# se-hwan/landing-controller

Measured on AMD Instinct MI355X. Metric: landing NLPs solved/sec (SRBM, N=40, batch), higher is better.
Workload: dtype f64

## Files before the change

### landing-controller_amd/csrc/solver_capi.inc

```

namespace {

struct StageTab {
  std::vector<int> tg_ab, tg_start, tg_term, gm_start, gm_term, a_term, r_start, r_term;
  int nu;
  std::vector<std::array<int, 4>> cterm;
  std::vector<std::array<int, 4>> rterm;
  std::vector<unsigned long long> cloc;
  bool operator==(const StageTab& o) const {
    return nu == o.nu && tg_ab == o.tg_ab && tg_start == o.tg_start && tg_term == o.tg_term && gm_start == o.gm_start &&
           gm_term == o.gm_term && a_term == o.a_term && r_start == o.r_start && r_term == o.r_term && cloc == o.cloc;
  }
};

int w_index(const Layout& L, int k, long long c) {
  const int N = L.N;
  if (c >= L.x_X(k) && c < L.x_X(k) + 12) return (int)(c - L.x_X(k));
  if (c >= L.x_U(k) && c < L.x_U(k) + 24) { const int j = (int)(c - L.x_U(k)); return j < 12 ? 12 + j : 24 + (j - 12); }
  if (k < N - 1 && c >= L.x_U(k + 1) && c < L.x_U(k + 1) + 12) return 36 + (int)(c - L.x_U(k + 1));
  return -1;
}
int jpos(const Layout& L, int k, long long c, long long idx) {
  if (c >= L.x_X(k) && c < L.x_X(k) + 12) return landing::NZ_JX + (int)(idx - L.jx(k));
  if (c >= L.x_U(k) && c < L.x_U(k) + 24) return landing::NZ_JU + (int)(idx - L.ju(k));
// ... 89 lines not shown
      };
      for (int i = 0; i < 12; ++i) add_c(i, i, i);
      for (int l = 0; l < 4; ++l) for (int a = 0; a < 3; ++a) add_c(a, 12 + 3 * l + a, 12 + 3 * l + a);
      for (int j = 0; j < 12; ++j) add_c(12 + j, 12 + j, 24 + j);
      for (int j = 0; j < 12; ++j) add_c(24 + j, 24 + j, 36 + j);
    }
    T.tg_start.push_back(0);
    for (auto& kv : tg) {
      T.tg_ab.push_back(kv.first.first | (kv.first.second << 8));
      for (auto& t : kv.second) { T.tg_term.push_back(t[0]); T.tg_term.push_back(t[1]); T.tg_term.push_back(t[2]); }
      T.tg_start.push_back((int)T.tg_term.size() / 3);
    }
    T.gm_start.push_back(0);
    for (int a = 0; a < 48; ++a) {
      for (auto& t : gm[a]) { T.gm_term.push_back(t[0]); T.gm_term.push_back(t[1]); }
      T.gm_start.push_back((int)T.gm_term.size() / 2);
    }
    {
      const int base = k * landing::COND_STRIDE;
      if ((int)T.tg_ab.size() > landing::COND_GAM || (int)T.a_term.size() / 3 > landing::COND_STRIDE - landing::COND_AH) return -7;
      int slot = 0;
      for (auto& kv : tg) {
        for (size_t i = 0; i < kv.second.size(); ++i) {
          const auto& t = kv.second[i];
          const int dst = (i + 1 == kv.second.size()) ? base + slot : -1;
          if (t[0] < 0) T.cterm.push_back({-1, pos2idx.at(t[1]), -1, dst});
          else T.cterm.push_back({g0 + t[0], pos2idx.at(t[1]), pos2idx.at(t[2]), dst});
        }
        ++slot;
      }
      for (int a = 0; a < 48; ++a) {
        if (gm[a].empty()) { T.cterm.push_back({-3, 0, -1, base + landing::COND_GAM + a}); continue; }
        for (size_t i = 0; i < gm[a].size(); ++i)
          T.cterm.push_back({g0 + gm[a][i][0], pos2idx.at(gm[a][i][1]), -1, (i + 1 == gm[a].size()) ? base + landing::COND_GAM + a : -1});
      }
      for (size_t i = 0; i < T.a_term.size() / 3; ++i) T.cterm.push_back({-2, pos2idx.at(T.a_term[3 * i]), -1, base + landing::COND_AH + (int)i});
    }
    for (auto& t : T.cterm) {
      int sa = 0, oa = 0, sb = 0, ob = 0;
      const bool has_b = t[2] >= 0;
      if (t[0] != -3 && !encode_jh(L, k, t[1], sa, oa)) return -9;
      if (has_b && !encode_jh(L, k, t[2], sb, ob)) return -9;
      const int rtype = t[0] >= 0 ? 0 : (t[0] == -1 ? 1 : (t[0] == -2 ? 2 : 3));
      const int rowq = t[0] >= 0 ? t[0] - g0 : 0;
      if (rowq < 0 || rowq >= 128) return -9;
      const int dstl = t[3] >= 0 ? t[3] - k * landing::COND_STRIDE : 0;
      if (dstl < 0 || dstl >= 1024) return -9;
      T.cloc.push_back(landing::cterm_pack(sa, oa, sb, ob, has_b, rowq, rtype, dstl, t[3] >= 0));
    }
    for (int ab : T.tg_ab) pat_g[k].insert(ab);
    for (size_t i = 0; i < T.a_term.size() / 3; ++i) pat_a[k].insert(T.a_term[3 * i + 1] * 64 + T.a_term[3 * i + 2]);
    for (auto& t : T.rterm) { rterms.push_back(t[0]); rterms.push_back(t[1]); rterms.push_back(t[2]); rterms.push_back(t[3]); }
    T.cterm.clear(); T.rterm.clear();
    int id = -1;
    for (size_t u = 0; u < uniq.size(); ++u) if (uniq[u] == T) { id = (int)u; break; }
    if (id < 0) { id = (int)uniq.size(); uniq.push_back(T); }
    which[k] = id;
  }
  int zero_each = 0;
  for (int k = N - 2; k >= 0; --k)
    if (!std::includes(pat_g[k].begin(), pat_g[k].end(), pat_g[k + 1].begin(), pat_g[k + 1].end()) ||
        !std::includes(pat_a[k].begin(), pat_a[k].end(), pat_a[k + 1].begin(), pat_a[k + 1].end())) zero_each = 1;
  if (zero_each) return -8;
  data.clear();
  std::vector<int> off(uniq.size());
  for (size_t u = 0; u < uniq.size(); ++u) {
    const StageTab& T = uniq[u];
    off[u] = (int)data.size();
    const int h = (int)data.size();
    data.resize(data.size() + 16, 0);
    auto put = [&](const std::vector<int>& v) { const int o = (int)data.size(); data.insert(data.end(), v.begin(), v.end()); return o; };
    data[h + 0] = (int)T.tg_ab.size();
    data[h + 1] = put(T.tg_ab); data[h + 2] = put(T.tg_start); data[h + 3] = put(T.tg_term);
    data[h + 4] = put(T.gm_start); data[h + 5] = put(T.gm_term);
    data[h + 6] = (int)T.a_term.size() / 3; data[h + 7] = put(T.a_term);
    data[h + 8] = put(T.r_start); data[h + 9] = put(T.r_term);
    data[h + 10] = T.nu;
    data[h + 11] = zero_each;
  }
  for (int k = 0; k < N; ++k) stage_tab[k] = off[which[k]];
  {
    using landing::Lds;
    const int NTH = landing::SOLVER_THREADS;
    const int oG = (int)offsetof(Lds, G), oGam = (int)offsetof(Lds, gam), oAh = (int)offsetof(Lds, Ah), oCx = (int)offsetof(Lds, jhl), oCarry = (int)offsetof(Lds, carry), oDump = (int)offsetof(Lds, dump);
    auto cx = [&](int pos) { return oCx + 8 * pos; };
    int ch = 0;
    for (size_t u = 0; u < uniq.size(); ++u) ch = std::max(ch, ((int)uniq[u].cloc.size() + NTH - 1) / NTH);
    struct Piece { std::vector<std::array<int, 3>> ops; int d; bool ah; };
    std::vector<std::vector<std::vector<unsigned long long>>> lists(uniq.size(), std::vector<std::vector<unsigned long long>>(NTH));
    ccomb.assign(uniq.size() * (size_t)NTH, 0ull);
    c_ml = 0;
    for (size_t u = 0; u < uniq.size(); ++u) {
      const StageTab& T = uniq[u];
      const auto& v = T.cloc; const int n = (int)v.size();
      if (n == 0 || !landing::cterm_closes(v[n - 1])) return -11;
      std::vector<Piece> pieces, cur;
      int nslot = 0, ncomb = 0;
      Piece pc_; pc_.d = 0; pc_.ah = false;
      for (int i = 0; i < n; ++i) {
        const unsigned lo = (unsigned)v[i], hi = (unsigned)(v[i] >> 32);
        const int pa = (int)(lo & 2047u), pb0 = (int)((lo >> 11) & 2047u), rowq = (int)((lo >> 23) & 127u), rtype = (int)(lo >> 30), dst = (int)(hi & 1023u);
        const bool has_b = (lo >> 22) & 1u, closes = landing::cterm_closes(v[i]);
        const int pb = has_b ? pb0 : landing::CX_ONE;
        const int pc = rtype == 0 ? landing::CX_SR + rowq + (has_b ? 0 : 104) : (rtype == 1 ? landing::CX_ONE : (rtype == 2 ? landing::CX_MONE : landing::CX_ZERO));
        if (i % ch == 0 && !pc_.ops.empty()) { cur.push_back(pc_); pc_.ops.clear(); }
        pc_.ops.push_back({cx(pa), cx(pb), cx(pc)});
        if (!closes) continue;
        int d; bool ah = false;
        if (dst < landing::COND_GAM) {
          if (dst >= (int)T.tg_ab.size()) return -12;
          const int a0 = T.tg_ab[dst] & 255, b0 = T.tg_ab[dst] >> 8;
          if (a0 >= 48 || b0 >= 48) return -12;
          d = oG + 8 * (std::min(a0, b0) * landing::GS + std::max(a0, b0));
        } else if (dst < landing::COND_AH) d = oGam + 8 * (dst - landing::COND_GAM);
        else {
          const int q = dst - landing::COND_AH;
          if (3 * q + 2 >= (int)T.a_term.size()) return -12;
          d = oAh + 8 * (T.a_term[3 * q + 1] * landing::YS + T.a_term[3 * q + 2]); ah = true;
        }
        cur.push_back(pc_); pc_.ops.clear();
        if (cur.size() == 1) { cur[0].d = d; cur[0].ah = ah; pieces.push_back(cur[0]); }
        else {
          if (cur.size() > 7 || nslot + (int)cur.size() > landing::ASM_NSLOT || ncomb >= NTH) return -13;
          ccomb[u * NTH + ncomb++] = landing::acomb_pack((int)cur.size(), oCarry + 8 * nslot, d, ah);
          for (auto& q : cur) { q.d = oCarry + 8 * nslot; q.ah = false; ++nslot; pieces.push_back(q); }
        }
        cur.clear();
      }
      std::vector<int> order(pieces.size());
      for (size_t i = 0; i < order.size(); ++i) order[i] = (int)i;
      std::stable_sort(order.begin(), order.end(), [&](int x, int y) { return pieces[x].ops.size() > pieces[y].ops.size(); });
      std::vector<int> load(NTH, 0);
      for (int di : order) {
        const int l = (int)(std::min_element(load.begin(), load.end()) - load.begin());
        const Piece& q = pieces[di];
        for (size_t i = 0; i < q.ops.size(); ++i) {
          const bool lastt = i + 1 == q.ops.size();
          lists[u][l].push_back(landing::aterm_pack(q.ops[i][0], q.ops[i][1], q.ops[i][2], lastt ? q.d : oDump + 8 * (l & 63), !lastt, lastt && q.ah));
        }
        load[l] += (int)q.ops.size();
      }
      c_ml = std::max(c_ml, *std::max_element(load.begin(), load.end()));
    }
    c_ml = (c_ml + landing::ATAB_TB - 1) / landing::ATAB_TB * landing::ATAB_TB;
    if (c_ml > landing::ATAB_LTMAX) return -10;
    ctab.assign(uniq.size() * (size_t)c_ml * NTH, 0ull);
    for (size_t u = 0; u < uniq.size(); ++u)
      for (int l = 0; l < NTH; ++l)
        for (int j = 0; j < c_ml; ++j)
          ctab[(u * c_ml + j) * NTH + l] = j < (int)lists[u][l].size() ? lists[u][l][j]
                                           : landing::aterm_pack(cx(landing::CX_ZERO), cx(landing::CX_ONE), cx(landing::CX_ONE), oDump + 8 * (l & 63), true, false);
    ctype.assign(N, 0);
    std::vector<int> cnt(uniq.size(), 0);
    for (int k = 0; k < N; ++k) { ctype[k] = which[k]; cnt[which[k]]++; }
    c_mid = (int)(std::max_element(cnt.begin(), cnt.end()) - cnt.begin());
  }
  auto chunk_at = [](const std::vector<int>& terms, int dstcol, std::vector<int>& start) {
    const int n = (int)terms.size() / 4, NTH = landing::SOLVER_THREADS;
    start.assign(NTH + 1, n);
    start[0] = 0;
    for (int t = 1; t < NTH; ++t) {
      int want = (int)((long long)n * t / NTH);
      if (want < start[t - 1]) want = start[t - 1];
      while (want < n && want > 0 && terms[4 * (want - 1) + dstcol] < 0) ++want;
      start[t] = want;
    }
  };
  chunk_at(rterms, 2, rstart);
  auto interleave = [](std::vector<int>& terms, std::vector<int>& start, const std::array<int, 4>& pad) {
    const int NTH = landing::SOLVER_THREADS;
    int maxlen = 0;
    for (int t = 0; t < NTH; ++t) maxlen = std::max(maxlen, start[t + 1] - start[t]);
    std::vector<int> out((size_t)maxlen * NTH * 4);
    for (int j = 0; j < maxlen; ++j) for (int t = 0; t < NTH; ++t) {
      const int e = start[t] + j;
      for (int q = 0; q < 4; ++q) out[((size_t)j * NTH + t) * 4 + q] = (e < start[t + 1]) ? terms[4 * (size_t)e + q] : pad[q];
    }
    terms.swap(out);
    start.assign(1, maxlen);
  };
  for (size_t i = 0; i < rterms.size() / 4; ++i) rterms[4 * i + 3] = 1;
  interleave(rterms, rstart, {0, 0, -1, 0});
  {
    const size_t n = rterms.size() / 4;
    std::vector<int> packed(2 * n);
    for (size_t i = 0; i < n; ++i) {
      const int ij = rterms[4 * i], ix = rterms[4 * i + 1], ir = rterms[4 * i + 2], valid = rterms[4 * i + 3];
      if (ij < 0 || ij > 0xffff || ix < 0 || ix > 0xffff || ir > 0xffff) return -18;
      const unsigned long long rec = (unsigned long long)ij | ((unsigned long long)ix << 16) | ((unsigned long long)(ir >= 0 ? ir : 0) << 32) |
                                     ((unsigned long long)(ir >= 0 ? 1 : 0) << 48) | ((unsigned long long)(valid ? 1 : 0) << 49);
      memcpy(&packed[2 * i], &rec, 8);
    }
    rterms.swap(packed);
  }
  return 0;
}

// ... 614 lines not shown
```

### landing-controller_amd/csrc/solver_kernels.hip

```cpp
#include <hip/hip_runtime.h>
#include <math.h>
#include <type_traits>

#include "../../include/landing_nlp.h"
#include "ipm_core.hpp"


namespace landing {

constexpr int NZ_JX = 0, NZ_JU = 157, NZ_JUN = 385, NZ_HX = 613, NZ_HU = 642, NZ_HUN = 802, NZ_TOT = 962;
constexpr int GS = 49;
constexpr int PS = 25;
constexpr int YS = 37;
constexpr int RIC_K = 0, RIC_KAP = 576, RIC_MT = 600, RIC_MV = 888, RIC_PX = 900, RIC_PV = 1188, RIC_STRIDE = 1200;
constexpr int RIC_FWD0 = 288, RIC_FWDN = 612;
constexpr int FILT_CAP = 64;
constexpr int SOLVER_NMAX = 96;
constexpr int ES = 26;
constexpr int SOLVER_THREADS = 256;
constexpr int COND_GAM = 480, COND_AH = 528, COND_STRIDE = 704;
constexpr int RCG = 36;
constexpr int RUNC = 48;

constexpr int CTAB_MLMAX = 6;
// ... 10 lines not shown
constexpr int ASM_NSLOT = 512;

constexpr int EXIT_REC = 8;
inline size_t member_stride(const Layout& L) {
  return (size_t)4 * L.nx + (size_t)20 * L.ng + L.nnz_jac + L.nnz_hess + (size_t)L.N * RUNC + (size_t)(L.N + 1) * RIC_STRIDE + (size_t)L.N * RCG + EXIT_REC;
}

enum { PH_EVAL = 0, PH_ERR, PH_SIGRHO, PH_BACK, PH_FWD, PH_DUAL, PH_LS, PH_ACCEPT, PH_NFACT, PH_NTRIAL, PH_NITER, PH_NSTAGE_OK, PH_B_ASM, PH_NSTAGE, PH_B_ELIM, PH_B_POST,
       PH_COUNT = 16 };
#define PROF_ADD(slot, tstart) do { if (SH.prof_on) { const long long n_ = (long long)wall_clock64(); if (threadIdx.x == 0) { SH.prof[slot] += (double)(n_ - (tstart)); (tstart) = n_; } } } while (0)

enum { EMU_ACC_FAST = 0, EMU_ACC_FAST_CLIP, EMU_ACC_FIRST_REJECTED, EMU_ACC_BACKTRACK, EMU_ACC_CORR, EMU_ACC_FALLBACK, EMU_ACC_FEAS, EMU_ACC_N };
#ifndef __HIPCC__
constexpr int EMU_ACC_MAXB = 64;
static int emu_acc[EMU_ACC_MAXB][EMU_ACC_N];
#define LANDING_EMU_COUNT(m, what) do { if ((m) < EMU_ACC_MAXB) emu_acc[m][what]++; } while (0)
static int emu_fused_on = 1;
#define LANDING_EMU_FUSED_ON (emu_fused_on != 0)
extern "C" void landing_emu_set_fused(int on) { emu_fused_on = on; }
extern "C" int landing_emu_accept_counts(int m, int* counts) {
  if (m < 0 || m >= EMU_ACC_MAXB || !counts) return -1;
  for (int i = 0; i < EMU_ACC_N; ++i) counts[i] = emu_acc[m][i];
  return 0;
}
#else
#define LANDING_EMU_COUNT(m, what) ((void)0)
#define LANDING_EMU_FUSED_ON true
#endif

struct SolveArgs {
  Layout L; int B; landing_solver_opts o; double* prof;
  const double* p; const double* x0;
  double* x_out; double* f_out; double* lam_out; int* status; int* iters; double* kkt;
  double* ws; size_t ws_stride;
  const unsigned long long* rterm; int rlen;
  const unsigned long long* ctab; const int* ctype; int c_ml, c_mid;
  const unsigned long long* ccomb;
  const int* edge_map;
  const int* order;
};

struct MemberMem {
  double *x, *xt, *dx, *gx;
  double *g, *gt, *s, *ds, *zL, *zU, *y, *yn, *sig, *rho;
  double *J, *H, *Hc, *ric, *cond;
  double *en, *ep, *wn, *wp;
  double *sig2, *rho2, *s2, *zL2, *zU2, *y2;
};
constexpr int MEMBER_MEM_PTRS = 29;
static_assert(sizeof(MemberMem) == MEMBER_MEM_PTRS * sizeof(double*) && std::is_standard_layout<MemberMem>::value && std::is_trivially_copyable<MemberMem>::value,
              "live_mem() walks MemberMem as an array of double*: nothing but double* members");

__device__ __forceinline__ MemberMem carve(const Layout& L, double* w) {
  MemberMem M;
  M.x = w; w += L.nx; M.xt = w; w += L.nx; M.dx = w; w += L.nx; M.gx = w; w += L.nx;
  M.g = w; w += L.ng; M.gt = w; w += L.ng; M.s = w; w += L.ng; M.ds = w; w += L.ng;
  M.zL = w; w += L.ng; M.zU = w; w += L.ng;
  M.y = w; w += L.ng; M.yn = w; w += L.ng;
  M.sig = w; w += L.ng; M.rho = w; w += L.ng;
  M.J = w; w += L.nnz_jac; M.H = w; w += L.nnz_hess; M.Hc = w; w += (size_t)L.N * RUNC; M.ric = w; w += (size_t)(L.N + 1) * RIC_STRIDE; M.cond = w; w += (size_t)L.N * RCG;
  M.en = w; w += L.ng; M.ep = w; w += L.ng; M.wn = w; w += L.ng; M.wp = w; w += L.ng;
  M.sig2 = w; w += L.ng; M.rho2 = w; w += L.ng;
  M.s2 = w; w += L.ng; M.zL2 = w; w += L.ng; M.zU2 = w; w += L.ng; M.y2 = w;
  return M;
}

__host__ __device__ __forceinline__ void mem_accept_swap(MemberMem& M) {
  double* t;
#define LANDING_SWAP(a, b) t = M.a; M.a = M.b; M.b = t
  LANDING_SWAP(s, s2); LANDING_SWAP(zL, zL2); LANDING_SWAP(zU, zU2); LANDING_SWAP(y, y2); LANDING_SWAP(sig, sig2); LANDING_SWAP(rho, rho2);
  LANDING_SWAP(g, gt); LANDING_SWAP(x, xt);
#undef LANDING_SWAP
}


constexpr int FWD_DXL_NMAX = 64;
constexpr int XCH = 112 * 4;
static_assert(2 * XCH >= 24 * YS, "A1 also holds Y (24 x YS)");
struct Lds {
  double G[48 * GS];
  double P[24 * PS];
  double A1[2 * XCH];
  double Ah[2 * 12 * YS];
  double gam[48], pv[24], q[24], bv[2 * 12], sig[24], w[48], dinv[24];
  double red[(SOLVER_THREADS / 64) * 9];
  double filt_th[FILT_CAP], filt_ph[FILT_CAP];
  double prof[32];
  int flag;
  int segb[SOLVER_NMAX * 8];
  double carry[ASM_NSLOT];
  double rcl[RCG];
  double jhl[CX_LEN];
  double dump[64];
  const unsigned long long* ctab; const unsigned long long* ccomb; int c_ml, c_mid, rc_on;
  double bnd_lb[36 + 2 * 104], bnd_ub[36 + 2 * 104];
  MemberMem M; Layout L; const double* p; int prof_on;
  IpmCtl ks;
  int clip_now, jamrun, action, fact_failed;
  int first_trial, fast;
  double nxt[6];
  unsigned long long atab_mid[ATAB_LTMAX * SOLVER_THREADS];
  unsigned long long acomb_mid[SOLVER_THREADS];
};
__shared__ Lds SH;
__device__ __forceinline__ MemberMem live_mem() {
  MemberMem M = SH.M;
#if defined(__HIP_DEVICE_COMPILE__)
  double** q = reinterpret_cast<double**>(&M);
#pragma unroll
  for (int i = 0; i < MEMBER_MEM_PTRS; ++i) {
    const unsigned long long a = (unsigned long long)q[i];
    const unsigned lo = (unsigned)__builtin_amdgcn_readfirstlane((int)(unsigned)a), hi = (unsigned)__builtin_amdgcn_readfirstlane((int)(unsigned)(a >> 32));
    q[i] = (double*)((unsigned long long)lo | ((unsigned long long)hi << 32));
  }
#endif
  return M;
}
static_assert(36 * FWD_DXL_NMAX + 12 <= 24 * PS + 2 * XCH + 2 * 12 * YS && offsetof(Lds, A1) == offsetof(Lds, P) + sizeof(double) * 24 * PS && offsetof(Lds, Ah) == offsetof(Lds, A1) + sizeof(double) * 2 * XCH,
              "dx (x layout, N <= FWD_DXL_NMAX) fits the adjacent arrays [P | A1 | A^] (forward_pass / row_products)");
static_assert(offsetof(Lds, atab_mid) <= 65528, "the assembly tables address G, A^, gamma, cx, the partial sums and the dump slots with 16-bit byte offsets");
__host__ __device__ inline unsigned long long aterm_pack(int pa, int pb, int pc, int d, bool keep, bool ah) {
  const unsigned lo = (unsigned)pa | ((unsigned)pb << 16);
  const unsigned hi = (unsigned)pc | (((unsigned)d | (keep ? 1u : 0u) | (ah ? 2u : 0u)) << 16);
  return (unsigned long long)lo | ((unsigned long long)hi << 32);
}
__host__ __device__ inline unsigned long long acomb_pack(int n, int s0, int d, bool ah) {
  return (unsigned long long)((unsigned)n | ((unsigned)s0 << 16)) | ((unsigned long long)((unsigned)d | (ah ? 2u : 0u)) << 32);
}

template <int KT, class FA, class FB>
__device__ __forceinline__ f64x4 mfma_tile(f64x4 c, FA fa, FB fb) {
  const int l = threadIdx.x & 63, ij = l & 15, kq = l >> 4;
#pragma unroll
  for (int kt = 0; kt < KT; ++kt) c = __builtin_amdgcn_mfma_f64_16x16x4f64(fa(ij, kt * 4 + kq), fb(kt * 4 + kq, ij), c, 0, 0, 0);
  return c;
}

__device__ __forceinline__ double fast_rcp(double d) {
  double i = __builtin_amdgcn_rcp(d);
  i = fma(i, fma(-d, i, 1.0), i);
  return fma(i, fma(-d, i, 1.0), i);
}

__device__ __forceinline__ double lane_bcast(double v, int src) {
  const int hi = __builtin_amdgcn_readlane(__double2hiint(v), src);
  const int lo = __builtin_amdgcn_readlane(__double2loint(v), src);
  return __hiloint2double(hi, lo);
}

template <int NU>
__device__ __noinline__ void gauss_jordan_wave(const double* G, const double* gam, double* Kl, double* kl, int* flag) {
  const int lane = threadIdx.x;
  double col[NU];
  const bool isUU = lane < NU, isUS = lane >= NU && lane < NU + 24, isG = lane == NU + 24;
  {
    const double* src = isG ? gam + 24 : G + 24 * GS + (isUU ? 24 + lane : (isUS ? lane - NU : 0));
    const int stride = isG ? 1 : GS;
#pragma unroll
    for (int i = 0; i < NU; ++i) col[i] = src[i * stride];
  }
  bool ok = true;
#pragma unroll 1
  for (int j = 0; j < NU; ++j) {
    const double d = lane_bcast(col[0], j);
    if (!(d > 0.0) || !(d < 1e300)) ok = false;
    double inv = __builtin_amdgcn_rcp(d);
    inv = fma(inv, fma(-d, inv, 1.0), inv);
    inv = fma(inv, fma(-d, inv, 1.0), inv);
    const double pj = col[0] * inv;
    double m[NU];
#pragma unroll
    for (int i = 1; i < NU; ++i) m[i] = lane_bcast(col[i], j);
    __builtin_amdgcn_sched_barrier(0);
#pragma unroll
    for (int i = 1; i < NU; ++i) col[i - 1] = fma(-m[i], pj, col[i]);
    col[NU - 1] = pj;
  }
  if (isUS) {
#pragma unroll
    for (int i = 0; i < NU; ++i) Kl[i * 24 + (lane - NU)] = col[i];
  }
  if (isG) {
#pragma unroll
    for (int i = 0; i < NU; ++i) kl[i] = col[i];
  }
  if (lane == 0) *flag = ok ? 1 : 0;
}

constexpr int ASM_SEG_LEN[7] = {NZ_JU - NZ_JX, NZ_JUN - NZ_JU, NZ_HX - NZ_JUN, NZ_HU - NZ_HX, NZ_HUN - NZ_HU, NZ_TOT - NZ_HUN, RUNC};
constexpr int ASM_SEG_POS[7] = {NZ_JX, NZ_JU, NZ_JUN, NZ_HX, NZ_HU, NZ_HUN, NZ_TOT};
static_assert(NZ_JUN - NZ_JU <= SOLVER_THREADS && 2 * 104 <= SOLVER_THREADS, "one load per thread and segment");
struct AsmRegs { double jh[7], sr, g, rc; };
__device__ __forceinline__ void asm_issue(int k, AsmRegs& R) {
  const Lds& S = SH;
  const MemberMem& M = S.M;
  const int tid = threadIdx.x, ng = S.L.ng;
  landing_gptr JH = (landing_gptr)M.J;
  landing_gptr SR = (landing_gptr)M.sig;
  const int* sb = S.segb + k * 8;
  const int g0 = S.L.g_stage(k);
#pragma unroll
  for (int sgm = 0; sgm < 7; ++sgm) R.jh[sgm] = JH[sb[sgm] + (tid < ASM_SEG_LEN[sgm] ? tid : 0)];
  R.sr = SR[tid < 104 ? g0 + tid : (tid < 208 ? ng + g0 + tid - 104 : 0)];
  R.g = ((landing_gptr)M.g)[g0 + (tid < 12 ? tid : 0)];
  R.rc = 0.0;
  if (S.rc_on) R.rc = ((landing_gptr)M.cond)[(size_t)k * RCG + (tid < RCG ? tid : 0)];
}
__device__ __forceinline__ void asm_copy(const AsmRegs& R) {
  Lds& S = SH;
  const int tid = threadIdx.x;
#pragma unroll
  for (int sgm = 0; sgm < 7; ++sgm) if (tid < ASM_SEG_LEN[sgm]) S.jhl[ASM_SEG_POS[sgm] + tid] = R.jh[sgm];
  if (tid < 208) S.jhl[CX_SR + tid] = R.sr;
}
__device__ __forceinline__ void asm_terms(int k, int nb, const AsmRegs& R) {
  Lds& S = SH;
  const int tid = threadIdx.x, LT = S.c_ml, tp = S.segb[k * 8 + 7];
  char* const lds0 = reinterpret_cast<char*>(&S);
  const unsigned ahoff = nb ? (unsigned)(12 * YS * sizeof(double)) : 0u;
  const bool mid = (tp == S.c_mid);
  const unsigned long long* gt = S.ctab + (size_t)tp * LT * SOLVER_THREADS;
  double acc = 0.0;
  for (int j0 = 0; j0 < LT; j0 += ATAB_TB) {
    unsigned long long t[ATAB_TB];
    if (mid) {
#pragma unroll
      for (int u = 0; u < ATAB_TB; ++u) t[u] = S.atab_mid[(j0 + u) * SOLVER_THREADS + tid];
    } else {
#pragma unroll
      for (int u = 0; u < ATAB_TB; ++u) t[u] = gt[(j0 + u) * SOLVER_THREADS + tid];
    }
    double a[ATAB_TB], b[ATAB_TB], c[ATAB_TB];
#pragma unroll
    for (int u = 0; u < ATAB_TB; ++u) {
      const unsigned lo = (unsigned)t[u], hi = (unsigned)(t[u] >> 32);
      a[u] = *reinterpret_cast<const double*>(lds0 + (lo & 0xffffu)); b[u] = *reinterpret_cast<const double*>(lds0 + (lo >> 16)); c[u] = *reinterpret_cast<const double*>(lds0 + (hi & 0xffffu));
    }
#pragma unroll
    for (int u = 0; u < ATAB_TB; ++u) {
      const unsigned dd = (unsigned)(t[u] >> 48);
      acc += a[u] * b[u] * c[u];
      *reinterpret_cast<double*>(lds0 + ((dd & 0xfff8u) + ((dd & 2u) ? ahoff : 0u))) = acc;
      acc = (dd & 1u) ? acc : 0.0;
    }
  }
  if (tid < 12) { const int i = tid; S.bv[nb * 12 + (i < 6 ? i : (i < 9 ? i + 3 : i - 3))] = -R.g; }
  if (tid < RCG) S.rcl[tid] = R.rc;
}
__device__ __forceinline__ void asm_combine(int k, int nb) {
  Lds& S = SH;
  const int tid = threadIdx.x, tp = S.segb[k * 8 + 7];
  const unsigned long long code = tp == S.c_mid ? S.acomb_mid[tid] : S.ccomb[tp * SOLVER_THREADS + tid];
  const unsigned lo = (unsigned)code, dd = (unsigned)(code >> 32);
  const int n = (int)(lo & 7u);
  if (n > 0) {
    char* const lds0 = reinterpret_cast<char*>(&S);
    const double* sl = reinterpret_cast<const double*>(lds0 + (lo >> 16));
    double tot = 0.0;
    for (int i = 0; i < n; ++i) tot += sl[i];
    *reinterpret_cast<double*>(lds0 + ((dd & 0xfff8u) + ((dd & 2u) ? (nb ? (unsigned)(12 * YS * sizeof(double)) : 0u) : 0u))) = tot;
  }
}

#if defined(__HIP_DEVICE_COMPILE__)
typedef double __attribute__((address_space(1)))* landing_gptr_w;
#else
typedef double* landing_gptr_w;
#endif

template <int STEP>
__device__ __forceinline__ bool pivot_block_step(f64x4 (&T)[3], int ct, int lj, int lk, int c) {
  constexpr int OFF = 4 * STEP;
  static_assert((OFF >> 4) == ((OFF + 3) >> 4), "a pivot block lies inside one row tile");
  Lds& S = SH;
  constexpr int RTB = OFF >> 4, R0 = (OFF & 15) >> 2;
  constexpr int WSZ = 64 * 4;
  static_assert(WSZ + 48 * 4 <= XCH, "exchange buffer");
  double* W = S.A1 + (STEP & 1) * XCH;
  double* C = W + WSZ;
#pragma unroll
  for (int q = 0; q < 1; ++q) W[c * 4 + 4 * q + lk] = T[RTB][R0 + q];
  if (ct == RTB && lj >= (OFF & 15) && lj < (OFF & 15) + 4) {
#pragma unroll
    for (int rt = 0; rt < 3; ++rt)
#pragma unroll
      for (int r = 0; r < 4; ++r) C[(16 * rt + lk + 4 * r) * 4 + (lj - (OFF & 15))] = T[rt][r];
  }
  __syncthreads();
  double a[4][4];
#pragma unroll
  for (int i = 0; i < 4; ++i)
#pragma unroll
    for (int j = 0; j <= i; ++j) a[i][j] = C[(OFF + i) * 4 + j];
  double w[4];
#pragma unroll
  for (int i = 0; i < 4; ++i) w[i] = W[c * 4 + i];
  double am[3];
#pragma unroll
  for (int rt = 0; rt < 3; ++rt) { const int row = 16 * rt + lj; const double cv = C[row * 4 + lk]; am[rt] = (row >= OFF && row < OFF + 4) ? 0.0 : cv; }
  auto recip = [](double d) { double i = __builtin_amdgcn_rcp(d); i = fma(i, fma(-d, i, 1.0), i); return fma(i, fma(-d, i, 1.0), i); };
  const double a00 = a[0][0], a10 = a[1][0], a11 = a[1][1], a20 = a[2][0], a21 = a[2][1], a22 = a[2][2], a30 = a[3][0], a31 = a[3][1], a32 = a[3][2], a33 = a[3][3];
  const double detA = fma(a00, a11, -a10 * a10), iA = recip(detA);
  const double e00 = fma(a20, a11, -a21 * a10) * iA, e01 = fma(a21, a00, -a20 * a10) * iA, e10 = fma(a30, a11, -a31 * a10) * iA, e11 = fma(a31, a00, -a30 * a10) * iA;
  const double s00 = fma(-e01, a21, fma(-e00, a20, a22)), s10 = fma(-e11, a21, fma(-e10, a20, a32)), s11 = fma(-e11, a31, fma(-e10, a30, a33));
  const double detS = fma(s00, s11, -s10 * s10), iS = recip(detS);
  unsigned hm = 0u;
  { const double piv[4] = {a00, detA, s00, detS};
#pragma unroll
    for (int j = 0; j < 4; ++j) { const unsigned h = (unsigned)__double2hiint(piv[j]) - 0x00100000u; hm = h > hm ? h : hm; } }
  const bool ok = hm < (0x7e37e43cu - 0x00100000u);
  auto solve = [&](const double (&wv)[4]) {
    const double t2 = fma(-e01, wv[1], fma(-e00, wv[0], wv[2])), t3 = fma(-e11, wv[1], fma(-e10, wv[0], wv[3]));
    const double r2 = fma(s11, t2, -s10 * t3) * iS, r3 = fma(s00, t3, -s10 * t2) * iS;
    const double q0 = fma(a11, wv[0], -a10 * wv[1]) * iA, q1 = fma(a00, wv[1], -a10 * wv[0]) * iA;
    const double r0 = fma(-e10, r3, fma(-e00, r2, q0)), r1 = fma(-e11, r3, fma(-e01, r2, q1));
    return lk == 0 ? r0 : (lk == 1 ? r1 : (lk == 2 ? r2 : r3));
  };
  const double R = solve(w);
  if (16 * ct + 16 > OFF) {
#pragma unroll
    for (int rt = 0; rt < 3; ++rt) T[rt] = __builtin_amdgcn_mfma_f64_16x16x4f64(am[rt], -R, T[rt], 0, 0, 0);
    T[RTB][R0] = R;
  }
  return ok;
}

template <int NU>
__device__ __noinline__ bool block_eliminate(double* __restrict__ rec, double delta, int k) {
  Lds& S = SH;
  constexpr int NR = NU + 24;
  const int tid = threadIdx.x, ct = tid >> 6, l = tid & 63, lj = l & 15, lk = l >> 4;
  const int c = 16 * ct + lj;
  const bool isg = (c == NR), live = (c <= NR);
  const int bcol = c < NU ? 24 + c : (c < NR ? c - NU : 0);
  const int cb = k & 1;
  const double* Ah = S.Ah + cb * (12 * YS);
  const double* bv = S.bv + cb * 12;
  f64x4 T[3];
  const double* const lds0 = reinterpret_cast<const double*>(&S);
  const int oG = (int)(offsetof(Lds, G) / sizeof(double)), oGam = (int)(offsetof(Lds, gam) / sizeof(double)), oP = (int)(offsetof(Lds, P) / sizeof(double)),
            oPv = (int)(offsetof(Lds, pv) / sizeof(double)), oAh = (int)(offsetof(Lds, Ah) / sizeof(double)) + cb * (12 * YS), oBv = (int)(offsetof(Lds, bv) / sizeof(double)) + cb * 12,
            oZ = (int)(offsetof(Lds, jhl) / sizeof(double)) + CX_ZERO;
  {
#pragma unroll
    for (int rt = 0; rt < 3; ++rt)
#pragma unroll
      for (int r = 0; r < 4; ++r) {
        const int rho = 16 * rt + lk + 4 * r;
        const int a = rho < NU ? 24 + rho : (rho < NR ? rho - NU : 0);
        const bool in = live && rho < NR;
        const double v = lds0[in ? (isg ? oGam + a : oG + (a < bcol ? a * GS + bcol : bcol * GS + a)) : oZ] + (rho == c ? delta : 0.0);
        T[rt][r] = in ? v : 0.0;
      }
    if (S.rc_on) {
#pragma unroll
      for (int rt = 0; rt < 3; ++rt)
#pragma unroll
        for (int r = 0; r < 4; ++r) {
          const int rho = 16 * rt + lk + 4 * r;
          const int a = rho < NU ? 24 + rho : (rho < NR ? rho - NU : 0);
          const double g = S.rcl[a < RCG ? a : 0];
          T[rt][r] += (isg && rho < NR && a < RCG) ? g : 0.0;
        }
    }
  }
  {
    const bool cplus = live && !isg && bcol >= 36;
    double be[3];
#pragma unroll
    for (int kt = 0; kt < 3; ++kt) be[kt] = lds0[isg ? oBv + 4 * kt + lk : ((live && bcol < 36) ? oAh + (4 * kt + lk) * YS + bcol : oZ)];
    double pa1[3], add1[3];
#pragma unroll
    for (int kt = 0; kt < 3; ++kt) pa1[kt] = lds0[oP + lj * PS + 4 * kt + lk];
#pragma unroll
    for (int r = 0; r < 3; ++r) { const int row = lk + 4 * r; add1[r] = lds0[cplus ? oP + row * PS + 12 + bcol - 36 : (isg ? oPv + row : oZ)]; }
    double av[3][3];
#pragma unroll
    for (int rt = 0; rt < 3; ++rt) {
      const int rho = 16 * rt + lj;
      const int a = rho < NU ? 24 + rho : (rho < NR ? rho - NU : 99);
#pragma unroll
      for (int kt = 0; kt < 3; ++kt) av[rt][kt] = lds0[a < 36 ? oAh + (4 * kt + lk) * YS + a : oZ];
    }
    double pa2[3], add2[3];
    if (NU == 24) {
#pragma unroll
      for (int kt = 0; kt < 3; ++kt) pa2[kt] = lds0[lj < 12 ? oP + (12 + lj) * PS + 4 * kt + lk : oZ];
#pragma unroll
      for (int r = 0; r < 3; ++r) { const int row = 12 + lk + 4 * r; add2[r] = lds0[cplus ? oP + row * PS + 12 + bcol - 36 : (isg ? oPv + row : oZ)]; }
    }
    f64x4 Y1 = {0.0, 0.0, 0.0, 0.0};
#pragma unroll
    for (int kt = 0; kt < 3; ++kt) Y1 = __builtin_amdgcn_mfma_f64_16x16x4f64(pa1[kt], be[kt], Y1, 0, 0, 0);
#pragma unroll
    for (int r = 0; r < 3; ++r) Y1[r] += add1[r];
#pragma unroll
    for (int rt = 0; rt < 3; ++rt)
#pragma unroll
      for (int kt = 0; kt < 3; ++kt) T[rt] = __builtin_amdgcn_mfma_f64_16x16x4f64(av[rt][kt], Y1[kt], T[rt], 0, 0, 0);
    if (NU == 24) {
      f64x4 Y2 = {0.0, 0.0, 0.0, 0.0};
#pragma unroll
      for (int kt = 0; kt < 3; ++kt) Y2 = __builtin_amdgcn_mfma_f64_16x16x4f64(pa2[kt], be[kt], Y2, 0, 0, 0);
#pragma unroll
      for (int r = 0; r < 3; ++r) Y2[r] += add2[r];
      T[0][3] += Y2[0]; T[1][0] += Y2[1]; T[1][1] += Y2[2];
    }
  }
  static_assert(NU == 12 || NU == 24, "3 or 6 block steps per stage");
  constexpr int SC = NU == 24 ? 3 : 1;
  AsmRegs nxt;
  const bool more = k > 0;
#define ASM_HOOK(step) do { if constexpr (SC == (step)) { if (more) asm_copy(nxt); } if constexpr (SC + 1 == (step)) { if (more) asm_terms(k - 1, cb ^ 1, nxt); } if constexpr (SC + 2 == (step)) { if (more) asm_combine(k - 1, cb ^ 1); } } while (0)
  bool ok = pivot_block_step<0>(T, ct, lj, lk, c);
  if (more) asm_issue(k - 1, nxt);
  ASM_HOOK(1);
  ok &= pivot_block_step<1>(T, ct, lj, lk, c);
  ASM_HOOK(2);
  ok &= pivot_block_step<2>(T, ct, lj, lk, c);
  ASM_HOOK(3);
  if constexpr (NU == 24) {
    ok &= pivot_block_step<3>(T, ct, lj, lk, c);
    ASM_HOOK(4);
    ok &= pivot_block_step<4>(T, ct, lj, lk, c);
    ASM_HOOK(5);
    ok &= pivot_block_step<5>(T, ct, lj, lk, c);
  }
#undef ASM_HOOK
  if (!ok) return false;
  {
    f64x4 Mq = {0.0, 0.0, 0.0, 0.0};
#pragma unroll
    for (int kt = 0; kt < 3; ++kt) {
      const double af = lds0[lj < 12 ? oAh + lj * YS + 24 + 4 * kt + lk : oZ];
      Mq = __builtin_amdgcn_mfma_f64_16x16x4f64(af, T[0][kt], Mq, 0, 0, 0);
    }
    if (c >= NU && c <= NR) {
#pragma unroll
      for (int r = 0; r < 3; ++r) {
        const int i = lk + 4 * r;
        if (c < NR) rec[RIC_MT + i * 24 + (c - NU)] = Ah[i * YS + (c - NU)] - Mq[r];
        else rec[RIC_MV + i] = bv[i] - Mq[r];
      }
    }
  }
  if (c >= NU && c <= NR) {
    const int sj = c - NU;
#pragma unroll
    for (int rt = 0; rt < 3; ++rt)
#pragma unroll
      for (int r = 0; r < 4; ++r) {
        const int rho = 16 * rt + lk + 4 * r;
        const double v = T[rt][r];
        if (rho < NU) {
          if (c < NR) rec[RIC_K + rho * 24 + sj] = v; else rec[RIC_KAP + rho] = v;
        } else if (rho < NR) {
          const int i = rho - NU;
          if (c < NR) { S.P[i * PS + sj] = v; if (i < 12) rec[RIC_PX + i * 24 + sj] = v; }
          else { S.pv[i] = v; if (i < 12) rec[RIC_PV + i] = v; }
        }
      }
  }
  return true;
}

template <int NU>
__device__ __forceinline__ bool riccati_step(double* rec, double delta, int k) {
  const bool ok = block_eliminate<NU>(rec, delta, k);
  __syncthreads();
  return ok;
}

__device__ __noinline__ bool riccati_backward(double delta) {
  Lds& S = SH;
  const Layout& L = S.L;
  const MemberMem& M = S.M;
  const double* p = S.p;
  const int N = L.N, lane = threadIdx.x, NT = blockDim.x;
  (void)p; (void)N; (void)lane; (void)NT;
  bool ok = true;
  int n_try = 0;
  for (int e = lane; e < 24 * PS; e += NT) S.P[e] = 0.0;
  __syncthreads();
  if (lane < 12) {
    const int i = lane;
    const int ra = i < 6 ? 12 + i : 24 + (i - 6), rb = i < 6 ? 18 + i : 30 + (i - 6);
    const double qn2 = S.ks.feas ? 0.0 : 2.0 * p[L.o_QN + i];
    S.P[i * PS + i] = qn2 + M.sig[ra] + M.sig[rb] + delta;
    S.pv[i] = qn2 * (M.x[12 * N + i] - p[12 * N + i]) + M.rho[ra] + M.rho[rb];
    double* rec = M.ric + (size_t)N * RIC_STRIDE;
    for (int j = 0; j < 24; ++j) rec[RIC_PX + i * 24 + j] = (j == i) ? S.P[i * PS + i] : 0.0;
    rec[RIC_PV + i] = S.pv[i];
  }
  for (int e = lane; e < 48 * GS; e += NT) S.G[e] = 0.0;
  for (int e = lane; e < 2 * 12 * YS; e += NT) S.Ah[e] = 0.0;
  if (lane < 24) S.pv[lane] = (lane < 12) ? S.pv[lane] : 0.0;
  __syncthreads();
  {
    AsmRegs first;
    asm_issue(N - 1, first);
    asm_copy(first);
    __syncthreads();
    asm_terms(N - 1, (N - 1) & 1, first);
    __syncthreads();
    asm_combine(N - 1, (N - 1) & 1);
  }
  __syncthreads();
  for (int k = N - 1; k >= 0 && ok; --k) {
    const bool last = (k == N - 1);
    long long tb_ = S.prof_on ? (long long)wall_clock64() : 0;
    double* rec = M.ric + (size_t)k * RIC_STRIDE;
    ok = last ? riccati_step<12>(rec, delta, k) : riccati_step<24>(rec, delta, k);
    ++n_try;
    PROF_ADD(PH_B_ELIM, tb_);
  }
  if (ok) {
    if (lane < 12) {
      const int i = lane;
      const double x0i = (i < 6) ? p[L.o_q_init + i] : p[L.o_qd_init + i - 6];
      S.sig[i] = x0i - M.x[i];
    }
    for (int e = lane; e < 144; e += NT) { const int i = e / 12, j = e % 12; S.G[(24 + i) * GS + 24 + j] = S.P[(12 + i) * PS + 12 + j]; }
    __syncthreads();
    if (lane < 12) {
      double v = S.pv[12 + lane];
      for (int t = 0; t < 12; ++t) v += S.P[(12 + lane) * PS + t] * S.sig[t];
      S.gam[24 + lane] = v;
    }
    __syncthreads();
    if (lane < 64) gauss_jordan_wave<12>(S.G, S.gam, S.A1, S.A1 + 24 * 24, &S.flag);
    __syncthreads();
    ok = S.flag != 0;
    ++n_try;
    if (ok) {
      if (lane < 12) S.sig[12 + lane] = -S.A1[24 * 24 + lane];
      __syncthreads();
    }
  }
  if (lane == 0) { S.prof[PH_NSTAGE] += (double)n_try; S.prof[PH_NSTAGE_OK] += (double)(ok ? n_try : n_try - 1); }
  __syncthreads();
  return ok;
}

__device__ __noinline__ void forward_pass() {
  Lds& S = SH;
  const Layout& L = S.L;
  const MemberMem& M = S.M;
  const int N = L.N, tid = threadIdx.x, NT = blockDim.x;
  double* sg = S.G;
  double* buf = S.jhl;
  double* buf1 = S.A1;
  static_assert(24 * (SOLVER_NMAX + 1) <= 48 * GS && RIC_FWDN <= NZ_TOT + RUNC && RIC_FWDN <= XCH * 2, "forward scratch fits");
  auto slot = [&](int k) { return (k & 1) ? buf1 : buf; };
  auto fetch = [&](int k, double (&r)[3]) {
    landing_gptr rec = (landing_gptr)(M.ric + (size_t)(k < N ? k : N - 1) * RIC_STRIDE + RIC_FWD0);
#pragma unroll
    for (int j = 0; j < 3; ++j) { const int e = tid + j * 256; r[j] = rec[e < RIC_FWDN ? e : RIC_FWDN - 1]; }
  };
  auto stash = [&](int k, const double (&r)[3]) {
    double* b = slot(k);
#pragma unroll
    for (int j = 0; j < 3; ++j) { const int e = tid + j * 256; if (k < N && e < RIC_FWDN) b[e] = r[j]; }
  };
  if (tid < 24) sg[tid] = S.sig[tid];
  double r0[3], r1[3], r2[3], r3[3];
  fetch(0, r0); fetch(1, r1); fetch(2, r2); fetch(3, r3);
  stash(0, r0); fetch(4, r0);
  __syncthreads();
  auto stage = [&](int k, double (&rn)[3]) {
    if (k < N) {
      const double* b = slot(k);
      const bool lastk = (k == N - 1);
      if (tid < 192) {
        const int r = tid >> 3, j = tid & 7;
        const double* row = (r < 12) ? b + 312 + r * 24 : b + (r - 12) * 24;
        const double* sk = sg + 24 * k;
        double acc = row[3 * j] * sk[3 * j] + row[3 * j + 1] * sk[3 * j + 1] + row[3 * j + 2] * sk[3 * j + 2];
        acc += __shfl_xor(acc, 1); acc += __shfl_xor(acc, 2); acc += __shfl_xor(acc, 4);
        if (j == 0) sg[24 * (k + 1) + r] = (r < 12) ? b[600 + r] + acc : (lastk ? 0.0 : -(b[300 + (r - 12)] + acc));
      }
    }
    stash(k + 1, rn);
    fetch(k + 5, rn);
    __syncthreads();
  };
  for (int k0 = 0; k0 < N; k0 += 4) {
    stage(k0, r1); stage(k0 + 1, r2); stage(k0 + 2, r3); stage(k0 + 3, r0);
  }
  double* const dxl = S.P;
  const bool use_dxl = N <= FWD_DXL_NMAX;
  for (int e = tid; e < 24 * (N + 1); e += NT) {
    const int k = e / 24, i = e % 24;
    if (i < 12) { M.dx[L.x_X(k) + i] = sg[e]; if (use_dxl) dxl[L.x_X(k) + i] = sg[e]; }
    else if (k < N) { M.dx[L.x_U(k) + (i - 12)] = sg[e]; if (use_dxl) dxl[L.x_U(k) + (i - 12)] = sg[e]; }
  }
  for (int e = tid; e < 24 * N; e += NT) {
    const int k = e / 24, h = e % 24, i = h % 12;
    const double* sk = sg + 24 * (h < 12 ? k : k + 1);
    if (h < 12) {
      landing_gptr rec = (landing_gptr)(M.ric + (size_t)k * RIC_STRIDE);
      double acc = rec[RIC_KAP + i];
#pragma unroll
      for (int t = 0; t < 24; ++t) acc += rec[RIC_K + i * 24 + t] * sk[t];
      M.dx[L.x_U(k) + 12 + i] = -acc;
      if (use_dxl) dxl[L.x_U(k) + 12 + i] = -acc;
    } else {
      landing_gptr recn = (landing_gptr)(M.ric + (size_t)(k + 1) * RIC_STRIDE);
      double acc = recn[RIC_PV + i];
// ... 719 lines not shown
```

Measured before the change: 20240.

## Store gamma, p and b in spare LDS columns and reorder G blocks

Moves the gamma, pv and bv vectors into the unused last columns of the G, P and Ah LDS matrices. It also permutes the G row/column order so that block_eliminate reads with uniform strided addressing instead of per-element branchy index selection. Record stores now use a readfirstlane-uniform base pointer and unsigned offsets. The aim is to cut address arithmetic and select overhead in the Riccati stage loop. The risk is that the host-side condensing offsets and the device layout must stay consistent, and the tail after backward elimination still reads S.gam.

```diff
diff --git a/landing-controller_amd/csrc/solver_capi.inc b/landing-controller_amd/csrc/solver_capi.inc
--- a/landing-controller_amd/csrc/solver_capi.inc
+++ b/landing-controller_amd/csrc/solver_capi.inc
@@ -195,8 +195,9 @@
   {
     using landing::Lds;
     const int NTH = landing::SOLVER_THREADS;
-    const int oG = (int)offsetof(Lds, G), oGam = (int)offsetof(Lds, gam), oAh = (int)offsetof(Lds, Ah), oCx = (int)offsetof(Lds, jhl), oCarry = (int)offsetof(Lds, carry), oDump = (int)offsetof(Lds, dump);
+    const int oG = (int)offsetof(Lds, G), oAh = (int)offsetof(Lds, Ah), oCx = (int)offsetof(Lds, jhl), oCarry = (int)offsetof(Lds, carry), oDump = (int)offsetof(Lds, dump);
     auto cx = [&](int pos) { return oCx + 8 * pos; };
+    auto gpos = [](int a) { return a < 24 ? a + 24 : a - 24; };
     int ch = 0;
     for (size_t u = 0; u < uniq.size(); ++u) ch = std::max(ch, ((int)uniq[u].cloc.size() + NTH - 1) / NTH);
     struct Piece { std::vector<std::array<int, 3>> ops; int d; bool ah; };
@@ -224,8 +225,8 @@
           if (dst >= (int)T.tg_ab.size()) return -12;
           const int a0 = T.tg_ab[dst] & 255, b0 = T.tg_ab[dst] >> 8;
           if (a0 >= 48 || b0 >= 48) return -12;
-          d = oG + 8 * (std::min(a0, b0) * landing::GS + std::max(a0, b0));
-        } else if (dst < landing::COND_AH) d = oGam + 8 * (dst - landing::COND_GAM);
+          d = oG + 8 * (std::min(gpos(a0), gpos(b0)) * landing::GS + std::max(gpos(a0), gpos(b0)));
+        } else if (dst < landing::COND_AH) d = oG + 8 * (gpos(dst - landing::COND_GAM) * landing::GS + landing::G_GAMMA);
         else {
           const int q = dst - landing::COND_AH;
           if (3 * q + 2 >= (int)T.a_term.size()) return -12;
diff --git a/landing-controller_amd/csrc/solver_kernels.hip b/landing-controller_amd/csrc/solver_kernels.hip
--- a/landing-controller_amd/csrc/solver_kernels.hip
+++ b/landing-controller_amd/csrc/solver_kernels.hip
@@ -116,7 +116,7 @@
   double P[24 * PS];
   double A1[2 * XCH];
   double Ah[2 * 12 * YS];
-  double gam[48], pv[24], q[24], bv[2 * 12], sig[24], w[48], dinv[24];
+  double gam[48], q[24], sig[24], w[48], dinv[24];
   double red[(SOLVER_THREADS / 64) * 9];
   double filt_th[FILT_CAP], filt_ph[FILT_CAP];
   double prof[32];
@@ -278,7 +278,7 @@
       acc = (dd & 1u) ? acc : 0.0;
     }
   }
-  if (tid < 12) { const int i = tid; S.bv[nb * 12 + (i < 6 ? i : (i < 9 ? i + 3 : i - 3))] = -R.g; }
+  if (tid < 12) { const int i = tid; S.Ah[nb * (12 * YS) + (i < 6 ? i : (i < 9 ? i + 3 : i - 3)) * YS + (YS - 1)] = -R.g; }
   if (tid < RCG) S.rcl[tid] = R.rc;
 }
 __device__ __forceinline__ void asm_combine(int k, int nb) {
@@ -301,6 +301,15 @@
 #else
 typedef double* landing_gptr_w;
 #endif
+__device__ __forceinline__ landing_gptr_w uniform_record(double* rec) {
+#if defined(__HIP_DEVICE_COMPILE__)
+  const unsigned long long a = (unsigned long long)rec;
+  const unsigned lo = (unsigned)__builtin_amdgcn_readfirstlane((int)(unsigned)a), hi = (unsigned)__builtin_amdgcn_readfirstlane((int)(unsigned)(a >> 32));
+  return (landing_gptr_w)((unsigned long long)lo | ((unsigned long long)hi << 32));
+#else
+  return rec;
+#endif
+}
 
 template <int STEP>
 __device__ __forceinline__ bool pivot_block_step(f64x4 (&T)[3], int ct, int lj, int lk, int c) {
@@ -359,69 +368,86 @@
   return ok;
 }
 
+constexpr int G_GAMMA = GS - 1, P_PV = PS - 1, AH_B = YS - 1;
+static_assert(G_GAMMA == 48 && P_PV == 24 && AH_B == 36, "spare columns of G / P / A^ hold gamma / p / b");
 template <int NU>
-__device__ __noinline__ bool block_eliminate(double* __restrict__ rec, double delta, int k) {
+__device__ __noinline__ bool block_eliminate(double* __restrict__ rec_, double delta, int k) {
   Lds& S = SH;
   constexpr int NR = NU + 24;
   const int tid = threadIdx.x, ct = tid >> 6, l = tid & 63, lj = l & 15, lk = l >> 4;
   const int c = 16 * ct + lj;
   const bool isg = (c == NR), live = (c <= NR);
-  const int bcol = c < NU ? 24 + c : (c < NR ? c - NU : 0);
   const int cb = k & 1;
-  const double* Ah = S.Ah + cb * (12 * YS);
-  const double* bv = S.bv + cb * 12;
   f64x4 T[3];
   const double* const lds0 = reinterpret_cast<const double*>(&S);
-  const int oG = (int)(offsetof(Lds, G) / sizeof(double)), oGam = (int)(offsetof(Lds, gam) / sizeof(double)), oP = (int)(offsetof(Lds, P) / sizeof(double)),
-            oPv = (int)(offsetof(Lds, pv) / sizeof(double)), oAh = (int)(offsetof(Lds, Ah) / sizeof(double)) + cb * (12 * YS), oBv = (int)(offsetof(Lds, bv) / sizeof(double)) + cb * 12,
-            oZ = (int)(offsetof(Lds, jhl) / sizeof(double)) + CX_ZERO;
+  constexpr int oG = (int)(offsetof(Lds, G) / sizeof(double)), oP = (int)(offsetof(Lds, P) / sizeof(double));
+  const int oAh = (int)(offsetof(Lds, Ah) / sizeof(double)) + cb * (12 * YS);
+  const int cl = c < NR ? c : NR;
+  const int cp = NU == 24 ? cl : (cl < NU ? cl : cl + (24 - NU));
+  const bool ym = live && (c < 12 || c >= NU);
+  int ycol = c < NU ? c + 24 : c - NU;
+  ycol = ym ? (isg ? AH_B : ycol) : 0;
+  const bool pm = live && c >= 12 && (c < NU || isg);
+  const int pcol = pm ? (isg ? P_PV : c) : 0;
   {
+    const int gb = oG + cp + lk * GS, cd = cp - lk, cm = c - lk;
 #pragma unroll
     for (int rt = 0; rt < 3; ++rt)
 #pragma unroll
       for (int r = 0; r < 4; ++r) {
-        const int rho = 16 * rt + lk + 4 * r;
-        const int a = rho < NU ? 24 + rho : (rho < NR ? rho - NU : 0);
-        const bool in = live && rho < NR;
-        const double v = lds0[in ? (isg ? oGam + a : oG + (a < bcol ? a * GS + bcol : bcol * GS + a)) : oZ] + (rho == c ? delta : 0.0);
-        T[rt][r] = in ? v : 0.0;
+        const int rb = 16 * rt + 4 * r;
+        if (rb < NR) {
+          const int rp = NU == 24 ? rb : (rb < NU ? rb : rb + (24 - NU));
+          const int m = rp < cd ? rp : cd;
+          const double v = lds0[gb + rp + (GS - 1) * m] + (cm == rb ? delta : 0.0);
+          T[rt][r] = live ? v : 0.0;
+        } else T[rt][r] = 0.0;
       }
     if (S.rc_on) {
 #pragma unroll
       for (int rt = 0; rt < 3; ++rt)
 #pragma unroll
         for (int r = 0; r < 4; ++r) {
-          const int rho = 16 * rt + lk + 4 * r;
-          const int a = rho < NU ? 24 + rho : (rho < NR ? rho - NU : 0);
-          const double g = S.rcl[a < RCG ? a : 0];
-          T[rt][r] += (isg && rho < NR && a < RCG) ? g : 0.0;
+          const int rb = 16 * rt + 4 * r;
+          if (rb < NR) {
+            const int ab = rb < NU ? 24 + rb : rb - NU;
+            static_assert(RCG % 4 == 0 && NU % 4 == 0, "a group of four rows lies on one side of every border");
+            const double g = ab < RCG ? S.rcl[ab + lk] : 0.0;
+            T[rt][r] += isg ? g : 0.0;
+          }
         }
     }
   }
   {
-    const bool cplus = live && !isg && bcol >= 36;
     double be[3];
-#pragma unroll
-    for (int kt = 0; kt < 3; ++kt) be[kt] = lds0[isg ? oBv + 4 * kt + lk : ((live && bcol < 36) ? oAh + (4 * kt + lk) * YS + bcol : oZ)];
+    {
+      const int yb = oAh + lk * YS + ycol;
+#pragma unroll
+      for (int kt = 0; kt < 3; ++kt) { const double v = lds0[yb + 4 * kt * YS]; be[kt] = ym ? v : 0.0; }
+    }
     double pa1[3], add1[3];
 #pragma unroll
     for (int kt = 0; kt < 3; ++kt) pa1[kt] = lds0[oP + lj * PS + 4 * kt + lk];
-#pragma unroll
-    for (int r = 0; r < 3; ++r) { const int row = lk + 4 * r; add1[r] = lds0[cplus ? oP + row * PS + 12 + bcol - 36 : (isg ? oPv + row : oZ)]; }
+    const int pb = oP + lk * PS + pcol;
+#pragma unroll
+    for (int r = 0; r < 3; ++r) { const double v = lds0[pb + 4 * r * PS]; add1[r] = pm ? v : 0.0; }
     double av[3][3];
 #pragma unroll
     for (int rt = 0; rt < 3; ++rt) {
       const int rho = 16 * rt + lj;
-      const int a = rho < NU ? 24 + rho : (rho < NR ? rho - NU : 99);
-#pragma unroll
-      for (int kt = 0; kt < 3; ++kt) av[rt][kt] = lds0[a < 36 ? oAh + (4 * kt + lk) * YS + a : oZ];
+      const int a = rho < NU ? 24 + rho : (rho < NR ? rho - NU : 36);
+      const bool am = a < 36;
+      const int ab = oAh + lk * YS + (am ? a : 0);
+#pragma unroll
+      for (int kt = 0; kt < 3; ++kt) { const double v = lds0[ab + 4 * kt * YS]; av[rt][kt] = am ? v : 0.0; }
     }
     double pa2[3], add2[3];
     if (NU == 24) {
-#pragma unroll
-      for (int kt = 0; kt < 3; ++kt) pa2[kt] = lds0[lj < 12 ? oP + (12 + lj) * PS + 4 * kt + lk : oZ];
-#pragma unroll
-      for (int r = 0; r < 3; ++r) { const int row = 12 + lk + 4 * r; add2[r] = lds0[cplus ? oP + row * PS + 12 + bcol - 36 : (isg ? oPv + row : oZ)]; }
+      const int p2 = oP + (12 + (lj < 12 ? lj : 11)) * PS + lk;
+#pragma unroll
+      for (int kt = 0; kt < 3; ++kt) pa2[kt] = lds0[p2 + 4 * kt];
+#pragma unroll
+      for (int r = 0; r < 3; ++r) { const double v = lds0[pb + (12 + 4 * r) * PS]; add2[r] = pm ? v : 0.0; }
     }
     f64x4 Y1 = {0.0, 0.0, 0.0, 0.0};
 #pragma unroll
@@ -462,36 +488,32 @@
   }
 #undef ASM_HOOK
   if (!ok) return false;
+  f64x4 Mq = {0.0, 0.0, 0.0, 0.0};
   {
-    f64x4 Mq = {0.0, 0.0, 0.0, 0.0};
-#pragma unroll
-    for (int kt = 0; kt < 3; ++kt) {
-      const double af = lds0[lj < 12 ? oAh + lj * YS + 24 + 4 * kt + lk : oZ];
-      Mq = __builtin_amdgcn_mfma_f64_16x16x4f64(af, T[0][kt], Mq, 0, 0, 0);
-    }
-    if (c >= NU && c <= NR) {
-#pragma unroll
-      for (int r = 0; r < 3; ++r) {
-        const int i = lk + 4 * r;
-        if (c < NR) rec[RIC_MT + i * 24 + (c - NU)] = Ah[i * YS + (c - NU)] - Mq[r];
-        else rec[RIC_MV + i] = bv[i] - Mq[r];
-      }
-    }
+    const int fb = oAh + (lj < 12 ? lj : 11) * YS + 24 + lk;
+#pragma unroll
+    for (int kt = 0; kt < 3; ++kt) Mq = __builtin_amdgcn_mfma_f64_16x16x4f64(lds0[fb + 4 * kt], T[0][kt], Mq, 0, 0, 0);
   }
   if (c >= NU && c <= NR) {
-    const int sj = c - NU;
+    const unsigned sj = (unsigned)(c - NU), ulk = (unsigned)lk;
+    const unsigned rs = isg ? 1u : 24u;
+    const unsigned iK = (isg ? (unsigned)RIC_KAP : (unsigned)RIC_K + sj) + ulk * rs, iM = (isg ? (unsigned)RIC_MV : (unsigned)RIC_MT + sj) + ulk * rs,
+                   iP = (isg ? (unsigned)RIC_PV : (unsigned)RIC_PX + sj) + ulk * rs;
+    const int scol = isg ? AH_B : (int)sj, pcw = isg ? P_PV : (int)sj;
+    landing_gptr_w rec = uniform_record(rec_);
+    double* const Pw = S.P + lk * PS + pcw;
+#pragma unroll
+    for (int r = 0; r < 3; ++r) rec[iM + (unsigned)(4 * r) * rs] = lds0[oAh + (lk + 4 * r) * YS + scol] - Mq[r];
 #pragma unroll
     for (int rt = 0; rt < 3; ++rt)
 #pragma unroll
       for (int r = 0; r < 4; ++r) {
-        const int rho = 16 * rt + lk + 4 * r;
+        const int rb = 16 * rt + 4 * r;
         const double v = T[rt][r];
-        if (rho < NU) {
-          if (c < NR) rec[RIC_K + rho * 24 + sj] = v; else rec[RIC_KAP + rho] = v;
-        } else if (rho < NR) {
-          const int i = rho - NU;
-          if (c < NR) { S.P[i * PS + sj] = v; if (i < 12) rec[RIC_PX + i * 24 + sj] = v; }
-          else { S.pv[i] = v; if (i < 12) rec[RIC_PV + i] = v; }
+        if (rb < NU) rec[iK + (unsigned)rb * rs] = v;
+        else if (rb < NR) {
+          Pw[(rb - NU) * PS] = v;
+          if (rb - NU < 12) rec[iP + (unsigned)(rb - NU) * rs] = v;
         }
       }
   }
@@ -521,14 +543,13 @@
     const int ra = i < 6 ? 12 + i : 24 + (i - 6), rb = i < 6 ? 18 + i : 30 + (i - 6);
     const double qn2 = S.ks.feas ? 0.0 : 2.0 * p[L.o_QN + i];
     S.P[i * PS + i] = qn2 + M.sig[ra] + M.sig[rb] + delta;
-    S.pv[i] = qn2 * (M.x[12 * N + i] - p[12 * N + i]) + M.rho[ra] + M.rho[rb];
+    S.P[i * PS + P_PV] = qn2 * (M.x[12 * N + i] - p[12 * N + i]) + M.rho[ra] + M.rho[rb];
     double* rec = M.ric + (size_t)N * RIC_STRIDE;
     for (int j = 0; j < 24; ++j) rec[RIC_PX + i * 24 + j] = (j == i) ? S.P[i * PS + i] : 0.0;
-    rec[RIC_PV + i] = S.pv[i];
+    rec[RIC_PV + i] = S.P[i * PS + P_PV];
   }
   for (int e = lane; e < 48 * GS; e += NT) S.G[e] = 0.0;
   for (int e = lane; e < 2 * 12 * YS; e += NT) S.Ah[e] = 0.0;
-  if (lane < 24) S.pv[lane] = (lane < 12) ? S.pv[lane] : 0.0;
   __syncthreads();
   {
     AsmRegs first;
@@ -557,7 +578,7 @@
     for (int e = lane; e < 144; e += NT) { const int i = e / 12, j = e % 12; S.G[(24 + i) * GS + 24 + j] = S.P[(12 + i) * PS + 12 + j]; }
     __syncthreads();
     if (lane < 12) {
-      double v = S.pv[12 + lane];
+      double v = S.P[(12 + lane) * PS + P_PV];
       for (int t = 0; t < 12; ++t) v += S.P[(12 + lane) * PS + t] * S.sig[t];
       S.gam[24 + lane] = v;
     }
```

New measurement: 21850 (median of 6 runs). 1.08x the previous value.
